# omid-arhami/topolow

Hardware: AMD Instinct MI355X
Metric: relaxation iterations/sec (NxN pairs) (higher is better)
Workload: dtype f32

## Files before the change

### include/topolow_relax.h

```cpp
#ifndef TOPOLOW_RELAX_H
#define TOPOLOW_RELAX_H

#include <stddef.h>
#include <stdint.h>

#ifdef __cplusplus
extern "C" {
#endif

#define TOPOLOW_OK 0
#define TOPOLOW_ERR_TOO_FEW_POINTS 1
#define TOPOLOW_ERR_NONFINITE 2
#define TOPOLOW_ERR_BAD_ARGUMENT 3
#define TOPOLOW_ERR_NO_DEVICE 4
#define TOPOLOW_ERR_HIP 5
#define TOPOLOW_ERR_UNSUPPORTED 6
#define TOPOLOW_ERR_INTERRUPTED 7


#define TOPOLOW_SCHEDULE_AUTO 0
#define TOPOLOW_SCHEDULE_SLAB 1
#define TOPOLOW_SCHEDULE_GS 2

#define TOPOLOW_PRECISION_AUTO 0
// ... 380 lines not shown
int topolow_session_get_positions(topolow_session* s, double* positions, char* errbuf,
                                  size_t errlen);

int topolow_session_begin(topolow_session* s, int32_t n_iter, double k0, double cooling_rate,
                          double c_repulsion, double relative_epsilon,
                          int32_t convergence_window, int32_t convergence_check_freq,
                          uint64_t seed, int32_t slab_stages, char* errbuf, size_t errlen);
int topolow_session_enqueue(topolow_session* s, int32_t max_iters, int32_t* enqueued,
                            char* errbuf, size_t errlen);
int topolow_session_wait(topolow_session* s, char* errbuf, size_t errlen);
int topolow_session_sync(topolow_session* s, int32_t* iterations_run, int32_t* stopped,
                         double* last_mae, char* errbuf, size_t errlen);
int topolow_session_finish(topolow_session* s, double* positions_out, int32_t* converged,
                           int32_t* iterations, double* final_mae, double* final_k,
                           char* errbuf, size_t errlen);
int topolow_session_check_trace(topolow_session* s, double* out, int32_t max_checks, int32_t* n_checks);
int topolow_session_hold_out(topolow_session* s, const int32_t* pair_i, const int32_t* pair_j, int64_t n_pairs,
                             const int32_t* degrees, char* errbuf, size_t errlen);
int topolow_session_restore_held_out(topolow_session* s, const int32_t* degrees, char* errbuf, size_t errlen);
int topolow_session_score_pairs(topolow_session* s, const int32_t* pair_i, const int32_t* pair_j, const double* truth,
                                int64_t n_pairs, double* sum_abs, int64_t* count, char* errbuf, size_t errlen);
int topolow_session_set_profiling(topolow_session* s, int32_t enable);
int topolow_session_profile_fused(topolow_session* s, double* fused_ms, int64_t* fused_launches, char* errbuf,
                                  size_t errlen);
int topolow_session_profile_symmetric(topolow_session* s, double* plain_ms, int64_t* plain_iterations, double* fused_ms,
                                      int64_t* fused_iterations, char* errbuf, size_t errlen);
int topolow_session_profile(topolow_session* s, double* stage_ms, int64_t* stage_launches,
                            double* check_ms, int64_t* checks, char* errbuf, size_t errlen);
int topolow_session_set_stream(topolow_session* s, void* hip_stream, int32_t external);
void* topolow_session_stream(topolow_session* s);
int32_t topolow_session_uses_dense_mae(const topolow_session* s);
int64_t topolow_session_stage_launches(const topolow_session* s);
int64_t topolow_session_checks_in_apply(const topolow_session* s);
int64_t topolow_session_bytes_per_iteration(const topolow_session* s);

int topolow_session_set_schedule(topolow_session* s, int32_t schedule);
int64_t topolow_tilegs_pair_order(int32_t n, uint64_t seed, int32_t iter, int32_t* pairs_out);
int32_t topolow_session_position_rows(const topolow_session* s);
int32_t topolow_session_position_dim(const topolow_session* s);
int topolow_session_stage(topolow_session* s, const void* d_pos_in, void* d_pos_out,
                          int32_t iter, int32_t stage, int32_t n_stages, double k,
                          char* errbuf, size_t errlen);
int topolow_session_check_partial(topolow_session* s, const void* d_pos, double* d_out2, char* errbuf,
                                  size_t errlen);
int topolow_session_controller_step(topolow_session* s, const double* d_total2, const void* d_pos,
                                    int32_t iter1, double k_after, char* errbuf, size_t errlen);
int32_t topolow_session_can_fuse_checks(const topolow_session* s);
int topolow_session_stage_fused(topolow_session* s, const void* d_pos_in, void* d_pos_out, int32_t iter,
                                double k, double* d_out2, char* errbuf, size_t errlen);
int32_t topolow_symm_segment_rows(int32_t n, int32_t segment, int32_t n_segments, int32_t* row_first,
                                  int32_t* row_end);
int32_t topolow_session_symm_segment_eligible(const topolow_session* s, int32_t n_segments);
int32_t topolow_session_can_fuse_segment_checks(const topolow_session* s);
float* topolow_session_degree_terms(topolow_session* s);
int32_t topolow_session_has_thresholds(const topolow_session* s);
int topolow_session_symm_segment_build(topolow_session* s, int32_t segment, int32_t n_segments, const void* d_rows,
                                       int32_t row_first, int32_t n_rows, int32_t any_threshold, char* errbuf,
                                       size_t errlen);
float* topolow_session_symm_moves(topolow_session* s);
int topolow_session_symm_segment_sweep(topolow_session* s, const void* d_pos_in, int32_t iter, double k,
                                       double* d_out2, char* errbuf, size_t errlen);
int topolow_session_symm_segment_apply(topolow_session* s, const void* d_pos_in, void* d_pos_out, int32_t iter,
                                       char* errbuf, size_t errlen);
int topolow_session_first_nonfinite(topolow_session* s, int32_t* iteration);
int topolow_session_edge_error(topolow_session* s, const void* d_pos, double* sum,
                               int64_t* count, char* errbuf, size_t errlen);
// ... 64 lines not shown
```

### topolow_amd/_native.py

```python
from __future__ import annotations

import ctypes as C
import math
import os
from dataclasses import dataclass, field
from typing import Any, Dict, Optional

import numpy as np

_HERE = os.path.dirname(os.path.abspath(__file__))
LIB_PATH = os.path.join(_HERE, "csrc", "libtopolow_relax.so")

SCHEDULE_AUTO, SCHEDULE_SLAB, SCHEDULE_GS = 0, 1, 2
PRECISION_AUTO, PRECISION_F32, PRECISION_F64, PRECISION_F64_EXACT = 0, 1, 2, 3

FAR_F32 = 1.0e18

OK = 0
ERR_TOO_FEW_POINTS, ERR_NONFINITE, ERR_BAD_ARGUMENT, ERR_NO_DEVICE, ERR_HIP, ERR_UNSUPPORTED, \
    ERR_INTERRUPTED = 1, 2, 3, 4, 5, 6, 7


class NativeError(RuntimeError):

# ... 193 lines not shown
    "topolow_layout_prep_fit_hist2d": (INT, (vp, dp, I32, i64p, I64, I32, I32, dp, I32, I32, dp, I32, i64p, i64p, i64p, *ERR)),
    "topolow_layout_prep_fit_linear_bins": (INT, (vp, dp, I32, i64p, I64, I32, I32, F64, F64, I32, i64p, u64p, i64p, i64p,
                                                  *ERR)),
    "topolow_session_create": (INT, (vpp, I32, I32, I32, I32, I32, I32, *ERR)),
    "topolow_session_destroy": (None, (vp,)),
    "topolow_session_set_relabel": (INT, (vp, U64, *ERR)),
    "topolow_session_labels": (INT, (vp, ip)),
    "topolow_session_load_dense": (INT, (vp, dp, ip, ip, *ERR)),
    "topolow_session_load_coo": (INT, (vp, ip, ip, dp, ip, I64, ip, *ERR)),
    "topolow_session_encoded_ptr": (devp, (vp,)),
    "topolow_session_encoded_ld": (I32, (vp,)),
    "topolow_session_commit_encoded": (INT, (vp, ip, *ERR)),
    "topolow_session_set_edges": (INT, (vp, ip, ip, dp, ip, I64, *ERR)),
    "topolow_session_set_positions": (INT, (vp, dp, *ERR)),
    "topolow_session_get_positions": (INT, (vp, dp, *ERR)),
    "topolow_session_begin": (INT, (vp, I32, F64, F64, F64, F64, I32, I32, U64, I32, *ERR)),
    "topolow_session_enqueue": (INT, (vp, I32, ip, *ERR)),
    "topolow_session_wait": (INT, (vp, *ERR)),
    "topolow_session_sync": (INT, (vp, ip, ip, dp, *ERR)),
    "topolow_session_finish": (INT, (vp, dp, ip, ip, dp, dp, *ERR)),
    "topolow_session_check_trace": (INT, (vp, dp, I32, ip)),
    "topolow_session_hold_out": (INT, (vp, ip, ip, I64, ip, *ERR)),
    "topolow_session_restore_held_out": (INT, (vp, ip, *ERR)),
    "topolow_session_score_pairs": (INT, (vp, ip, ip, dp, I64, dp, i64p, *ERR)),
    "topolow_session_set_profiling": (INT, (vp, I32)),
    "topolow_session_profile_fused": (INT, (vp, dp, i64p, *ERR)),
    "topolow_session_profile_symmetric": (INT, (vp, dp, i64p, dp, i64p, *ERR)),
    "topolow_session_profile": (INT, (vp, dp, i64p, dp, i64p, *ERR)),
    "topolow_session_set_stream": (INT, (vp, vp, I32)),
    "topolow_session_stream": (devp, (vp,)),
    "topolow_session_uses_dense_mae": (I32, (vp,)),
    "topolow_session_stage_launches": (I64, (vp,)),
    "topolow_session_checks_in_apply": (I64, (vp,)),
    "topolow_session_bytes_per_iteration": (I64, (vp,)),
    "topolow_session_set_schedule": (INT, (vp, I32)),
    "topolow_tilegs_pair_order": (I64, (I32, U64, I32, ip)),
    "topolow_session_position_rows": (I32, (vp,)),
    "topolow_session_position_dim": (I32, (vp,)),
    "topolow_session_stage": (INT, (vp, devp, devp, I32, I32, I32, F64, *ERR)),
    "topolow_session_check_partial": (INT, (vp, devp, devp, *ERR)),
    "topolow_session_controller_step": (INT, (vp, devp, devp, I32, F64, *ERR)),
    "topolow_session_can_fuse_checks": (I32, (vp,)),
    "topolow_session_stage_fused": (INT, (vp, devp, devp, I32, F64, devp, *ERR)),
    "topolow_symm_segment_rows": (I32, (I32, I32, I32, ip, ip)),
    "topolow_session_symm_segment_eligible": (I32, (vp, I32)),
    "topolow_session_can_fuse_segment_checks": (I32, (vp,)),
    "topolow_session_degree_terms": (devp, (vp,)),
    "topolow_session_has_thresholds": (I32, (vp,)),
    "topolow_session_symm_segment_build": (INT, (vp, I32, I32, devp, I32, I32, I32, *ERR)),
    "topolow_session_symm_moves": (devp, (vp,)),
    "topolow_session_symm_segment_sweep": (INT, (vp, devp, I32, F64, devp, *ERR)),
    "topolow_session_symm_segment_apply": (INT, (vp, devp, devp, I32, *ERR)),
    "topolow_session_first_nonfinite": (INT, (vp, ip)),
    "topolow_session_edge_error": (INT, (vp, devp, dp, i64p, *ERR)),
    "topolow_shard_rows": (I32, (I32, I32, I32, ip, ip)),
    "topolow_optimize_layout_exact_sharded": (INT, (dp, I32, I32, dp, ip, ip, ip, ip, dp, ip, I64, I32, F64, F64, F64, F64,
                                                    I32, I32, I32, optionsp, dp, ip, ip, dp, dp, shard_statsp, *ERR)),
    "topolow_sessions_run_sharded": (INT, (vpp, I32, dp, I32, F64, F64, F64, F64, I32, I32, U64, I32, INTERRUPT_CB, vp, I32,
                                           dp, ip, ip, dp, dp, shard_statsp, *ERR)),
    "topolow_slab_plan": (I32, (I32, I32, U64, I32, ip, I32)),
    "topolow_slab_stages_for_k": (I32, (F64, I32)),
    "topolow_symm_stage_bounds": (I32, (I32, I32, ip)),
    "topolow_symm_stage_order": (I32, (U64, I32, I32, ip)),
    "topolow_symm_stage_rows": (I32, (I32, I32, I32, ip)),
    "topolow_symm_plan": (I32, (I32, I32, I32, I32, I32, I32, ip, I32, ip)),
    "topolow_session_symm_grid": (I32, (vp,)),
# ... 1101 lines not shown
        return out.values()

    def profile_symmetric(self):
        return self._profile(self.lib.topolow_session_profile_symmetric, 2)

    def profile_fused(self):
        return self._profile(self.lib.topolow_session_profile_fused, 1)

    def set_stream(self, hip_stream, external: bool = True):
        self.lib.topolow_session_set_stream(self._h, C.c_void_p(hip_stream or None),
                                            int(bool(external)))

    @property
    def stream(self) -> int:
        return int(self.lib.topolow_session_stream(self._h) or 0)

    @property
    def position_rows(self) -> int:
        return int(self.lib.topolow_session_position_rows(self._h))

    @property
    def uses_dense_mae(self) -> bool:
        return bool(self.lib.topolow_session_uses_dense_mae(self._h))

    @property
    def stage_launches(self) -> int:
        return int(self.lib.topolow_session_stage_launches(self._h))

    @property
    def checks_in_apply(self) -> int:
        return int(self.lib.topolow_session_checks_in_apply(self._h))

    @property
    def symm_grid(self) -> int:
        return int(self.lib.topolow_session_symm_grid(self._h))

    @property
    def bytes_per_iteration(self) -> int:
        return int(self.lib.topolow_session_bytes_per_iteration(self._h))

    def stage(self, d_pos_in: int, d_pos_out: int, it: int, stage: int, n_stages: int, k: float):
        _call(self.lib.topolow_session_stage, self._h, C.c_void_p(d_pos_in), C.c_void_p(d_pos_out), int(it), int(stage),
              int(n_stages), float(k), err=self._err)

    def check_partial(self, d_pos: int, d_out2: int):
        _call(self.lib.topolow_session_check_partial, self._h, C.c_void_p(d_pos), C.c_void_p(d_out2), err=self._err)

    def controller_step(self, d_total2: int, d_pos: int, iter1: int, k_after: float):
        _call(self.lib.topolow_session_controller_step, self._h, C.c_void_p(d_total2), C.c_void_p(d_pos), int(iter1),
              float(k_after), err=self._err)

    @property
    def can_fuse_checks(self) -> bool:
        return bool(self.lib.topolow_session_can_fuse_checks(self._h))

    def stage_fused(self, d_pos_in: int, d_pos_out: int, it: int, k: float, d_out2: int):
        _call(self.lib.topolow_session_stage_fused, self._h, C.c_void_p(d_pos_in), C.c_void_p(d_pos_out), int(it), float(k),
              C.c_void_p(d_out2), err=self._err)

    @property
    def degree_terms_ptr(self) -> int:
        return int(self.lib.topolow_session_degree_terms(self._h) or 0)

    @property
    def has_thresholds(self) -> bool:
        return bool(self.lib.topolow_session_has_thresholds(self._h))
# ... 35 lines not shown
```

### topolow_amd/csrc/relax_symm.h

```cpp
#pragma once

#include <hip/hip_runtime.h>
#include <algorithm>
#include <type_traits>
#include <vector>
#include "relax_common.h"
#include "relax_kernels.h"
#include "relax_symm_plan.h"

namespace topolow {

#ifndef TOPOLOW_SYM_MINW
#define TOPOLOW_SYM_MINW 2
#endif

typedef float symf2 __attribute__((ext_vector_type(2)));
#ifdef TOPOLOW_SYM_STAMPS
__device__ unsigned long long* g_sym_stamps = nullptr;
#endif

#define TL_SYM_DPP_ADD(v, ctrl) asm volatile("v_add_f32_dpp %0, %0, %0 " ctrl " row_mask:0xf bank_mask:0xf" : "+v"(v))
template <int NV>
__device__ __forceinline__ void sym_col_reduce(float (&first)[NV], float (&second)[NV]) {
#pragma unroll
// ... 263 lines not shown
#pragma unroll
        for (int d = 0; d < DIM; ++d) {
          dst[(2 * p) * DIM + d] = racc2[p][d].x;
          dst[(2 * p + 1) * DIM + d] = racc2[p][d].y;
        }
    }
    if constexpr (ERR) {
      double s = (double)err_unit;
#pragma unroll
      for (int m = 32; m >= 1; m >>= 1) s += __shfl_xor(s, m, 64);
      if constexpr (ANYTHR) {
#pragma unroll
        for (int m = 32; m >= 1; m >>= 1) cnt_unit2 += __shfl_xor(cnt_unit2, m, 64);
      }
      if (lane == 0) {
        part_sum[slot] = s;
        part_cnt[slot] = ANYTHR ? (unsigned long long)cnt_unit2 : (slot == 0 ? fixed_cnt : 0ull);
      }
    }
  }
#ifdef TOPOLOW_SYM_STAMPS
  if (lane == 0 && g_sym_stamps != nullptr) {
    g_sym_stamps[4 * gw] = __builtin_amdgcn_s_memtime() - stamp_c0;
    g_sym_stamps[4 * gw + 1] = stamp_r0;
    g_sym_stamps[4 * gw + 2] = __builtin_amdgcn_s_memrealtime();
    unsigned hw_id, xcc_id;
    asm volatile("s_getreg_b32 %0, hwreg(HW_REG_HW_ID)" : "=s"(hw_id));
    asm volatile("s_getreg_b32 %0, hwreg(HW_REG_XCC_ID)" : "=s"(xcc_id));
    g_sym_stamps[4 * gw + 3] = ((unsigned long long)xcc_id << 32) | hw_id;
  }
#endif
}

template <int DIM, typename real> struct SymReal;
template <int DIM> struct SymReal<DIM, float> {
  static constexpr int W = SymRec<DIM>::W;
  __device__ static float ks(double k, float g) { return (float)(2.0 * k) / (4.0f * g + (float)k); }
  __device__ static float cg(double c_rep, float g) { return (float)(0.5 * c_rep) / g; }
  __device__ static float far(int) { return kFarF32; }
};

struct SymApplyCheck {
  const double* part_sum = nullptr;
  const unsigned long long* part_cnt = nullptr;
  int n_parts = 0;
  const void* pos = nullptr;
  void* best0 = nullptr;
  void* best1 = nullptr;
  long long n_values = 0;
  int check_no = 0;
  int iter1 = 0;
  double k_after = 0.0;
  double* trace = nullptr;
  int trace_cap = 0;
  RunState* mailbox = nullptr;
};

#ifndef TL_APPLY_PARTS
#define TL_APPLY_PARTS 16
#endif
constexpr int kSymApplyParts = TL_APPLY_PARTS;

template <int DIM, typename real>
__global__ __launch_bounds__(32 * kSymApplyParts) void symm_apply_kernel(
    const real* __restrict__ rec, real* __restrict__ rec_next, real* __restrict__ pos_out, const float* __restrict__ gplus,
    const real* __restrict__ rowpart, const real* __restrict__ colpart, const int2* __restrict__ row_units, int n,
// ... 210 lines not shown
```

### topolow_amd/csrc/topolow_relax.hip

```cpp

#include "topolow_session.h"
#include "topolow_prep.h"
#include "relax_kernels.h"
#include "relax_exact.h"
#include "relax_tilegs.h"
#include "relax_symm.h"
#include "relax_symm64.h"
#include "relax_symm_wide.h"
#include "relax_cv.h"

namespace {

#define TL_DISPATCH_DIM(dim, FN, ...)                 \
  switch (dim) {                                      \
    case 1: FN<1>(__VA_ARGS__); break;                \
    case 2: FN<2>(__VA_ARGS__); break;                \
    case 3: FN<3>(__VA_ARGS__); break;                \
    case 4: FN<4>(__VA_ARGS__); break;                \
    case 5: FN<5>(__VA_ARGS__); break;                \
    case 6: FN<6>(__VA_ARGS__); break;                \
    case 7: FN<7>(__VA_ARGS__); break;                \
    case 8: FN<8>(__VA_ARGS__); break;                \
    case 9: FN<9>(__VA_ARGS__); break;                \
    case 10: FN<10>(__VA_ARGS__); break;              \
// ... 555 lines not shown
  return s->sym.holds == SymHolds::kTriangle;
}

template <int DIM>
void sym_records(topolow_session* s, const void* pin, void* rec, double k) {
  sym_real<DIM>(s, [&](auto r) {
    using real = decltype(r);
    hipLaunchKernelGGL((symm_records_kernel<DIM, real>), dim3((s->sym.npad + 255) / 256), dim3(256), 0, s->stream,
                       (const real*)pin, s->gplus.p, (real*)rec, s->n, s->sym.npad, k, s->c_rep);
  });
}

template <int DIM>
void sym_sweep(topolow_session* s, const SymPlanDev& plan, const void* rec, bool thr, bool err,
               unsigned long long block_cells, int col_row0, bool prio) {
  auto& y = s->sym;
  if (err && ((size_t)plan.n_units > s->part_sum.n || (size_t)plan.n_units > s->part_cnt.n))
    throw HipError{TOPOLOW_ERR_HIP, "symmetric sweep: the error partials are smaller than the plan's unit count"};
  sym_real<DIM>(s, [&](auto r) {
    using real = decltype(r);
    sym_sweep_instance<DIM, real>(thr, err, s->exact, [&](auto kern) {
      if constexpr (std::is_same<real, double>::value)
        hipLaunchKernelGGL(kern, dim3(y.grid), dim3(64 * kSymWaves), 0, s->stream, y.tenc.p, (const double*)rec,
                           plan.units.p, plan.runs.p, (double*)y.rowpart.p, (double*)y.colpart.p, y.npad, s->state.p,
                           col_row0, y.tdelta.p, s->part_sum.p, s->part_cnt.p, block_cells);
      else
        hipLaunchKernelGGL(kern, dim3(y.grid), dim3(64 * kSymWaves), 0, s->stream, y.tenc.p, (const float*)rec,
                           plan.units.p, plan.runs.p, (float*)y.rowpart.p, (float*)y.colpart.p, y.npad, s->state.p,
                           s->part_sum.p, s->part_cnt.p, block_cells, col_row0, prio && y.prio ? 1 : 0);
    });
  });
}

bool sym_fused_ok(const topolow_session* s) {
  if (!s->sym.delta_ready) return false;
  return !s->exact || (s->list_is_block && s->n_edges > 0 && s->sym.holds == SymHolds::kTriangle);
}

template <int DIM>
void sym_apply(topolow_session* s, const SymPlanDev& plan, const void* rec, void* rec_next, void* pout, double k_next,
               int iter, int rr_stages, int rr_stage, const PendingCheck* chk = nullptr, const void* pin = nullptr,
               int n_parts = 0) {
  auto& y = s->sym;
  SymApplyCheck ac;
  if (chk != nullptr) {
    ac.part_sum = s->part_sum.p;
    ac.part_cnt = s->part_cnt.p;
    ac.n_parts = n_parts;
    ac.pos = pin;
    ac.best0 = s->best[0].p;
    ac.best1 = s->best[1].p;
    ac.check_no = s->checks_launched;
    ac.n_values = (long long)s->n * s->dim;
    ac.iter1 = chk->iter1;
    ac.k_after = chk->k_after;
    ac.trace = s->trace_dev;
    ac.trace_cap = s->trace_cap;
    ac.mailbox = s->mailbox_dev;
  }
  sym_real<DIM>(s, [&](auto r) {
    using real = decltype(r);
    hipLaunchKernelGGL((symm_apply_kernel<DIM, real>), dim3(y.npad / kSymCols + (chk != nullptr ? 1 : 0)),
                       dim3(32 * kSymApplyParts), 0, s->stream,
                       (const real*)rec, (real*)rec_next, (real*)pout, s->gplus.p, (const real*)y.rowpart.p,
                       (const real*)y.colpart.p, plan.row_units.p, s->n, y.npad, k_next, s->c_rep, iter + 1, s->state.p,
                       rr_stages, rr_stage, ac);
  });
}

bool sym_rr_stages_ok(int S) { return S == 2 || S == 4 || S == 8; }
int sym_rr_log2(int S) { return S == 2 ? 1 : (S == 4 ? 2 : 3); }

SymPlan sym_rr_plan(int npad, int n_waves, int S, int st) {
  const int TR = npad / kSymRows;
  return relax_symm_plan_rows(npad, n_waves, [&](int R, int& j0, int& j1) { sym_rr_row(TR, S, st, R, j0, j1); });
}

bool sym_rr_available(topolow_session* s, int S) {
  auto& y = s->sym;
  if (!sym_rr_stages_ok(S) || y.holds != SymHolds::kTriangle) return false;
  const int TR = y.npad / kSymRows;
  if (TR < 2 * S) return false;
  if ((long long)TR * (TR + 1) / S < (long long)y.rr_min_tiles * y.grid * kSymWaves) return false;
  const int lg = sym_rr_log2(S);
  if (!y.rr[lg].empty()) return true;
  std::vector<SymPlanDev> plans(S);
  for (int st = 0; st < S; ++st) {
    const SymPlan hp = sym_rr_plan(y.npad, y.grid * kSymWaves, S, st);
    if (hp.units.size() * kSymRows * s->dim * s->real_size() > y.rowpart.n) return false;
    plans[st].load(hp);
  }
  y.rr[lg] = std::move(plans);
  return true;
}

template <int DIM>
void sym_iteration(topolow_session* s, const void* pin, void* pout, int iter, double k, bool err, int S = 0, int st = 0,
                   bool last = true, const PendingCheck* in_apply = nullptr) {
  auto& y = s->sym;
  const SymPlanDev& plan = S == 0 ? y.plan : y.rr[sym_rr_log2(S)][st];
  ProfScope prof(s, S > 0 ? &s->prof_stage : err ? &s->prof_sym_err : &s->prof_sym);
  if (err && s->precision == TOPOLOW_PRECISION_F64 && !sym_fused_ok(s))
    throw HipError{TOPOLOW_ERR_UNSUPPORTED, "symmetric sweep (f64): no delta tiles for a fused check"};
  if (y.rec_iter != iter) {
    for (int b = 0; b < 2; ++b)
      sym_records<DIM>(s, pin, y.rec[b].p, k);
    y.rec_cur = 0;
  }
  sym_sweep<DIM>(s, plan, y.rec[y.rec_cur].p, s->any_threshold, err, S == 0 ? s->block_cells : 0ull, 0, true);
  if (in_apply != nullptr && !(err && S == 0))
    throw HipError{TOPOLOW_ERR_BAD_ARGUMENT, "symmetric sweep: a check in the apply needs the ERR sweep of a one-stage iteration"};
  sym_apply<DIM>(s, plan, y.rec[y.rec_cur].p, y.rec[y.rec_cur ^ 1].p, pout, last ? k * (1.0 - s->cooling) : k, iter, S, st,
                 in_apply, pin, plan.n_units);
  HIP_TRY(hipGetLastError());
  y.rec_cur ^= 1;
  y.rec_iter = last ? iter + 1 : iter;
  if (err) s->fused_parts = plan.n_units;
  s->stage_launches += 1;
}

enum class SymForm { kRowOwner, kSweep, kStages };
SymForm sym_form(topolow_session* s, int n_stages) {
  if (n_stages == 1) return sym_eligible(s) && sym_available(s) ? SymForm::kSweep : SymForm::kRowOwner;
  return s->sym.two_stage && sym_rr_stages_ok(n_stages) && sym_eligible(s) && sym_available(s) &&
                 sym_rr_available(s, n_stages)
             ? SymForm::kStages
             : SymForm::kRowOwner;
}

int iteration_stages(const topolow_session* s, int iter, double k) {
  return slab_geom(s->n, s->fixed_stages > 0 ? s->fixed_stages : slab_stages_at(iter, k, s->dim)).n_stages;
}

bool check_after(const topolow_session* s, int iter) { return (iter + 1) % s->check_freq == 0 || iter == s->n_iter - 1; }

struct IterPlan {
  SlabGeom geo;
  SymForm form;
  int order[8];
};
IterPlan plan_iteration(topolow_session* s, int iter, double k) {
  IterPlan p;
  p.geo = slab_geom(s->n, iteration_stages(s, iter, k));
  p.form = sym_form(s, p.geo.n_stages);
  if (p.form == SymForm::kStages) sym_rr_order(s->seed, iter, p.geo.n_stages, p.order);
  return p;
}

int enqueue_stage(topolow_session* s, const IterPlan& p, int t, const void* pin, void* pout, int iter, double k,
                  const void* push, int n_push, bool err, const PendingCheck* in_apply = nullptr) {
  if (in_apply != nullptr && p.form != SymForm::kSweep)
    throw HipError{TOPOLOW_ERR_BAD_ARGUMENT, "a check in the apply needs a one-stage symmetric sweep"};
  if (p.form == SymForm::kRowOwner) {
    TL_DISPATCH_DIM(s->dim, launch_stage, s, pin, pout, s->state.p, slab_ranges(p.geo, s->seed, iter, t), iter + 1, k,
                    push, n_push, err);
    if (err) s->fused_parts = (s->rows() + CfgProd::ROWS - 1) / CfgProd::ROWS;
  } else if (p.form == SymForm::kSweep) {
    TL_DISPATCH_SYM(s->dim, sym_iteration, s, pin, pout, iter, k, err, 0, 0, true, in_apply);
  } else {
    const int S = p.geo.n_stages;
    TL_DISPATCH_SYM(s->dim, sym_iteration, s, pin, pout, iter, k, err, S, p.order[t], t == S - 1);
  }
  return err ? s->fused_parts : 0;
}

bool check_fusable(topolow_session* s, int n_stages) {
  if (s->precision == TOPOLOW_PRECISION_F64)
    return sym_form(s, 1) == SymForm::kSweep && sym_fused_ok(s) && n_stages == 1;
  return n_stages == 1 && (s->rows() % 2 == 0 || sym_form(s, 1) == SymForm::kSweep);
}

struct SymSegment {
  long long total, t0, t1;
  int r_first = -1, r_last = -1;
};
SymSegment sym_segment(int n, int b, int P) {
  SymSegment g;
  const int npad = (n + kSymRows - 1) & ~(kSymRows - 1), TR = npad / kSymRows;
  g.total = (long long)TR * (TR + 1);
  g.t0 = g.total * b / P;
  g.t1 = g.total * (b + 1) / P;
  (void)relax_symm_plan(npad, 1, g.t0, g.t1, &g.r_first, &g.r_last);
  return g;
}

bool sym_sharded_eligible(const std::vector<topolow_session*>& ss) {
  const char* e = getenv("TOPOLOW_SHARD_SYMMETRIC");
  if (e != nullptr && e[0] == '0') return false;
  const int P = (int)ss.size();
  if (P < 2) return false;
  const topolow_session* a = ss[0];
  const long long TR = ((a->n + kSymRows - 1) & ~(kSymRows - 1)) / kSymRows;
  if (TR * (TR + 1) < 8ll * P) return false;
  for (const topolow_session* s : ss)
// ... 101 lines not shown
  if (g.r_first >= 0 && (row_first > g.r_first * kSymRows ||
                         row_first + n_rows < std::min<long long>(s->n, (long long)(g.r_last + 1) * kSymRows)))
    throw HipError{TOPOLOW_ERR_BAD_ARGUMENT, "symm_segment_build: d_rows does not hold the rows of the segment's tiles"};
  sym_build<DIM>(s, {d_rows}, {row_first, row_first + n_rows}, any_thr, g.t0, g.t1);
  sym_install_segment<DIM>(s, SymHolds::kCallerSegment, any_thr, 1, 0, {0, s->n});
}

void launch_check(topolow_session* s, PendingCheck& pc, bool error_pass) {
  hipStream_t check_on = s->stream;
  if (pc.beside) {
    HIP_TRY(hipEventRecord(s->ev_iter_done, s->stream));
    HIP_TRY(hipStreamWaitEvent(s->check_stream, s->ev_iter_done, 0));
    check_on = s->check_stream;
  }
  {
    StreamScope on(s, check_on);
    ProfScope prof(s, &s->prof_check);
    if (error_pass) {
      TL_DISPATCH_DIM(s->dim, launch_edge_error, s, s->pos[pc.buf].p, s->state.p);
      launch_controller(s, s->pos[pc.buf].p, pc.iter1, pc.k_after);
    } else {
      launch_controller(s, s->pos[pc.buf].p, pc.iter1, pc.k_after, s->part_sum.p, s->part_cnt.p, s->fused_parts);
    }
  }
  if (pc.beside) HIP_TRY(hipEventRecord(s->ev_check_done, check_on));
  hipEvent_t e = take_event(s);
  HIP_TRY(hipEventRecord(e, check_on));
  s->pending.push_back(e);
  s->checks_launched += 1;
  poll_checks(s, 3);
  pc.active = false;
}

void check_went_in_apply(topolow_session* s, PendingCheck& pc) {
  s->checks_launched += 1;
  s->checks_in_apply += 1;
  pc.active = false;
  const volatile RunState* mb = s->mailbox;
  double asked = now_s();
  while (!mb->stopped && s->checks_launched - mb->n_checks > 3) {
    if (now_s() - asked < 1e-3) continue;
    if (hipStreamQuery(s->stream) != hipErrorNotReady) break;
    (void)hipGetLastError();
    asked = now_s();
  }
  if (mb->stopped) s->host_seen_stop = true;
}

void flush_pending_check(topolow_session* s) {
  if (s->pcheck.active) launch_check(s, s->pcheck, true);
}

int nonfinite_report(int first_nonfinite, int ran, bool stopped) {
  if (first_nonfinite == 0x7fffffff) return 0;
  const int t = ((first_nonfinite + 9) / 10) * 10;
  return t <= ran && !(stopped && t == ran) ? t : 0;
}


void edges_begin(topolow_session* s, int64_t n_edges) {
  s->n_edges = n_edges;
  s->cv.list_compacted = false;
  if (s->precision == TOPOLOW_PRECISION_F64) s->sym.invalidate();
  s->n_parts = edge_error_blocks(n_edges);
  s->dense_grid_x = (((s->n + 3) & ~3) + ErrCfg::CHUNK - 1) / ErrCfg::CHUNK;
  s->dense_grid_y = (s->rows() + kErrTileRows - 1) / kErrTileRows;
  s->dense_blocks = s->dense_grid_x * s->dense_grid_y;
  const int stage_blocks = (s->rows() + CfgProd::ROWS - 1) / CfgProd::ROWS;
  int parts = std::max({s->n_parts, s->dense_blocks, stage_blocks, s->sym.plan.n_units});
  for (const auto& plans : s->sym.rr)
    for (const auto& p : plans) parts = std::max(parts, p.n_units);
  s->part_sum.alloc(parts);
  s->part_cnt.alloc(parts);
  s->dense_mae = false;
  s->dense_parity = !(s->row_begin == 0 && s->row_end == s->n);
  s->list_is_block = false;
}

bool edge_mae_forced() {
  const char* force = getenv("TOPOLOW_EDGE_MAE");
  return force && atoi(force) != 0;
}

void block_fingerprint(topolow_session* s, unsigned long long h[2]) {
  DevBuf<unsigned long long> d_fp;
  d_fp.alloc(2);
  HIP_TRY(hipMemsetAsync(d_fp.p, 0, 16, s->stream));
  hipLaunchKernelGGL(upper_fingerprint_kernel, dim3(s->rows()), dim3(kThreads), 0, s->stream,
                     s->enc.p, s->n, s->row_begin, s->row_end, s->ld, s->dense_parity ? 1 : 0,
                     d_fp.p);
  HIP_TRY(hipGetLastError());
  HIP_TRY(hipStreamSynchronize(s->stream));
  HIP_TRY(hipMemcpy(h, d_fp.p, 16, hipMemcpyDeviceToHost));
}

void edges_decide(topolow_session* s, bool list_is_block) {
  s->list_is_block = list_is_block;
  s->dense_mae = list_is_block && s->dim <= kMaxTunedDim && s->precision == TOPOLOW_PRECISION_F32;
}

bool edges_placeholders(topolow_session* s) {
  if (!s->dense_mae) return false;
  s->ei.alloc(1); s->ej.alloc(1); s->ec.alloc(1); s->et.alloc(8);
  return true;
// ... 440 lines not shown
    s->device = dev;
    s->n = n;
    s->dim = kernel_dim(ndim);
    s->udim = ndim;
    s->row_begin = row_begin;
    s->row_end = row_end;
    s->ld = (n + kEncLdAlign - 1) & ~(kEncLdAlign - 1);
    s->precision = precision == TOPOLOW_PRECISION_F64 || exact ? TOPOLOW_PRECISION_F64 : TOPOLOW_PRECISION_F32;
    s->exact = exact;
    HIP_TRY(hipStreamCreateWithFlags(&s->own_stream, hipStreamNonBlocking));
    s->stream = s->own_stream;
    HIP_TRY(hipStreamCreateWithFlags(&s->check_stream, hipStreamNonBlocking));
    HIP_TRY(hipEventCreateWithFlags(&s->ev_iter_done, hipEventDisableTiming));
    HIP_TRY(hipEventCreateWithFlags(&s->ev_check_done, hipEventDisableTiming));
    const char* serial = getenv("TOPOLOW_SERIAL_CHECKS");
    s->serial_checks = serial != nullptr && serial[0] == '1';
    const char* fuse = getenv("TOPOLOW_FUSE_CHECKS");
    s->fuse_checks = !(fuse != nullptr && fuse[0] == '0');
    const char* in_apply = getenv("TOPOLOW_CHECK_IN_APPLY");
    s->check_in_apply = !(in_apply != nullptr && in_apply[0] == '0');
    const char* symm = getenv("TOPOLOW_SYMMETRIC");
    s->sym.allowed = !(symm != nullptr && symm[0] == '0');
    s->sym.forced = symm != nullptr && symm[0] == '1';
    const char* symm_min = getenv("TOPOLOW_SYMMETRIC_MIN_N");
    s->sym.min_n = symm_min != nullptr ? atoi(symm_min) : kSymMinPoints;
    const char* symm2 = getenv("TOPOLOW_SYMMETRIC_TWO_STAGE");
    s->sym.two_stage = !(symm2 != nullptr && symm2[0] == '0');
    const char* rr_min = getenv("TOPOLOW_SYMMETRIC_STAGE_MIN_TILES");
    if (rr_min != nullptr) s->sym.rr_min_tiles = std::max(0, atoi(rr_min));
    const char* sym_grid = getenv("TOPOLOW_SYMMETRIC_GRID");
    s->sym.grid_cap = sym_grid != nullptr ? std::max(0, atoi(sym_grid)) : 0;
    const char* sym_prio = getenv("TOPOLOW_SYM_PRIO");
    s->sym.prio = !(sym_prio != nullptr && sym_prio[0] == '0');
    s->enc.alloc((size_t)((s->rows() + kEncRowAlign - 1) / kEncRowAlign * kEncRowAlign) * s->ld);
    if (s->exact) s->denc.alloc(s->enc.n);
    const size_t pos_bytes = (size_t)s->pos_rows() * s->dim * s->real_size();
    for (auto& b : s->pos) b.alloc(pos_bytes);
    for (auto& b : s->best) b.alloc(pos_bytes);
    s->state.alloc(1);
    HIP_TRY(hipHostMalloc((void**)&s->mailbox, sizeof(RunState), hipHostMallocMapped));
    std::memset(s->mailbox, 0, sizeof(RunState));
    HIP_TRY(hipHostGetDevicePointer((void**)&s->mailbox_dev, s->mailbox, 0));
  });
  if (rc != TOPOLOW_OK) { delete s; return rc; }
  *out = s;
  return TOPOLOW_OK;
}

void topolow_session_destroy(topolow_session* s) {
  if (!s) return;
  (void)hipSetDevice(s->device);
  if (s->stream) (void)hipStreamSynchronize(s->stream);
  if (s->check_stream) (void)hipStreamSynchronize(s->check_stream);
#ifdef TOPOLOW_TUNING
  g_stamps.dump();
#endif
  delete s;
}

int topolow_session_set_relabel(topolow_session* s, uint64_t seed, char* errbuf, size_t errlen) {
  if (!s) return TOPOLOW_ERR_BAD_ARGUMENT;
  if (s->gplus.p || s->part_sum.p) {
    set_err(errbuf, errlen, "the relabelling must be chosen before targets, edges or positions are loaded");
    return TOPOLOW_ERR_BAD_ARGUMENT;
  }
  return guarded(errbuf, errlen, [&] {
// ... 206 lines not shown
  return guarded(errbuf, errlen, [&] {
    HIP_TRY(hipSetDevice(s->device));
    if (!s->gplus.p) throw HipError{TOPOLOW_ERR_BAD_ARGUMENT, "session has no targets loaded"};
    if (!s->part_sum.p) throw HipError{TOPOLOW_ERR_BAD_ARGUMENT, "session has no edge list"};
    HIP_TRY(hipStreamSynchronize(s->stream));
    HIP_TRY(hipStreamSynchronize(s->check_stream));
    for (hipEvent_t e : s->pending) s->event_pool.push_back(e);
    s->pending.clear();
    s->n_iter = n_iter;
    s->k0 = k0;
    s->cooling = cooling_rate;
    s->c_rep = c_repulsion;
    s->eps = relative_epsilon;
    s->window = convergence_window;
    s->check_freq = convergence_check_freq < 1 ? 10 : convergence_check_freq;
    {
      const int need = n_iter / s->check_freq + 2;
      if (need > s->trace_cap) {
        if (s->trace) { (void)hipHostFree(s->trace); s->trace = nullptr; s->trace_cap = 0; }
        HIP_TRY(hipHostMalloc((void**)&s->trace, sizeof(double) * 3 * (size_t)need, hipHostMallocMapped));
        HIP_TRY(hipHostGetDevicePointer((void**)&s->trace_dev, s->trace, 0));
        s->trace_cap = need;
      }
    }
    s->seed = seed;
    s->fixed_stages = slab_stages;
    s->iters_enqueued = 0;
    s->k_host = k0;
    s->host_seen_stop = false;
    s->held = -1;
    s->pcheck.active = false;
    s->checks_launched = 0;
    s->checks_in_apply = 0;
    s->sym.rec_iter = -1;
    s->began = true;
    s->in_run = true;
    RunState st;
    std::memset(&st, 0, sizeof st);
    st.ctl.init(k0, convergence_window, relative_epsilon);
    st.k_base = k0;
    st.cooling = cooling_rate;
    st.n_iter = n_iter;
    st.first_nonfinite = 0x7fffffff;
    *s->mailbox = st;
    HIP_TRY(hipMemcpyAsync(s->state.p, &st, sizeof st, hipMemcpyHostToDevice, s->stream));
    HIP_TRY(hipMemcpyAsync(s->best[0].p, s->pos[s->cur].p,
                           (size_t)s->pos_rows() * s->dim * s->real_size(), hipMemcpyDeviceToDevice,
                           s->stream));
    HIP_TRY(hipStreamSynchronize(s->stream));
  });
}

int topolow_session_enqueue(topolow_session* s, int32_t max_iters, int32_t* enqueued,
                            char* errbuf, size_t errlen) {
  if (!s || !s->began) return TOPOLOW_ERR_BAD_ARGUMENT;
  if (enqueued) *enqueued = 0;
  return guarded(errbuf, errlen, [&] {
    HIP_TRY(hipSetDevice(s->device));
    int done = 0;
    while (done < max_iters && s->iters_enqueued < s->n_iter && !s->host_seen_stop) {
      const int iter = s->iters_enqueued;
      if (s->schedule == TOPOLOW_SCHEDULE_GS) {
        TL_DISPATCH_DIM(s->dim, launch_tilegs_iteration, s, s->pos[s->cur].p, iter, s->k_host);
      } else {
        const IterPlan plan = plan_iteration(s, iter, s->k_host);
        const bool fuse_now = s->pcheck.active && check_fusable(s, plan.geo.n_stages);
        if (s->pcheck.active && !fuse_now) flush_pending_check(s);
        const bool in_apply = fuse_now && s->pcheck.in_apply && plan.form == SymForm::kSweep;
        for (int t = 0; t < plan.geo.n_stages; ++t) {
          int out = 0;
          while (out == s->cur || out == s->held) ++out;
          enqueue_stage(s, plan, t, s->pos[s->cur].p, s->pos[out].p, iter, s->k_host, nullptr, 0, fuse_now,
                        in_apply ? &s->pcheck : nullptr);
          s->cur = out;
        }
        if (in_apply) check_went_in_apply(s, s->pcheck);
        else if (fuse_now) launch_check(s, s->pcheck, false);
      }
      s->iters_enqueued = iter + 1;
      s->k_host *= (1.0 - s->cooling);
      ++done;
      if (check_after(s, iter)) {
        PendingCheck pc{true, iter + 1, s->k_host, s->cur};
        pc.beside = s->schedule == TOPOLOW_SCHEDULE_SLAB && s->stream == s->own_stream &&
                    !s->profiling && !s->serial_checks;
        if (s->check_in_apply && iter + 1 == s->n_iter) pc.beside = false;
        if (s->held >= 0) HIP_TRY(hipStreamWaitEvent(s->stream, s->ev_check_done, 0));
        const bool fuse = s->fuse_checks && s->schedule == TOPOLOW_SCHEDULE_SLAB && iter + 1 < s->n_iter &&
                          (s->dense_mae || s->precision == TOPOLOW_PRECISION_F64) &&
                          check_fusable(s, iteration_stages(s, iter + 1, s->k_host));
        if (pc.beside && fuse && s->check_in_apply && sym_form(s, 1) == SymForm::kSweep) {
          pc.in_apply = true;
          pc.beside = false;
        }
        s->held = pc.beside ? s->cur : -1;
        if (fuse) s->pcheck = pc;
        else launch_check(s, pc, true);
      }
      if (s->schedule == TOPOLOW_SCHEDULE_GS && (iter + 1) % 10 == 0)
        launch_tilegs_finite(s, s->pos[s->cur].p, iter + 1);
    }
    if (enqueued) *enqueued = done;
  });
}

int topolow_session_wait(topolow_session* s, char* errbuf, size_t errlen) {
  if (!s) return TOPOLOW_ERR_BAD_ARGUMENT;
  return guarded(errbuf, errlen, [&] {
    HIP_TRY(hipSetDevice(s->device));
    HIP_TRY(hipStreamSynchronize(s->stream));
    HIP_TRY(hipStreamSynchronize(s->check_stream));
  });
}

int topolow_session_sync(topolow_session* s, int32_t* iterations_run, int32_t* stopped,
                         double* last_mae, char* errbuf, size_t errlen) {
  if (!s) return TOPOLOW_ERR_BAD_ARGUMENT;
  return guarded(errbuf, errlen, [&] {
    HIP_TRY(hipSetDevice(s->device));
    flush_pending_check(s);
    HIP_TRY(hipStreamSynchronize(s->stream));
    HIP_TRY(hipStreamSynchronize(s->check_stream));
    poll_checks(s, 0);
    RunState st;
// ... 132 lines not shown
  (void)hipStreamSynchronize(s->stream);
  (void)hipStreamSynchronize(s->check_stream);
  s->stream = external ? (hipStream_t)hip_stream : s->own_stream;
  return TOPOLOW_OK;
}

void* topolow_session_stream(topolow_session* s) { return s ? (void*)s->stream : nullptr; }

int topolow_session_set_schedule(topolow_session* s, int32_t schedule) {
  if (!s || (schedule != TOPOLOW_SCHEDULE_SLAB && schedule != TOPOLOW_SCHEDULE_GS))
    return TOPOLOW_ERR_BAD_ARGUMENT;
  if (s->row_begin != 0 || s->row_end != s->n) return TOPOLOW_ERR_UNSUPPORTED;
  s->schedule = schedule;
  return TOPOLOW_OK;
}

int64_t topolow_tilegs_pair_order(int32_t n, uint64_t seed, int32_t iter, int32_t* pairs_out) {
  return tilegs_pair_order(n, seed, iter, pairs_out);
}

int32_t topolow_session_position_rows(const topolow_session* s) { return s ? s->pos_rows() : 0; }
int32_t topolow_session_position_dim(const topolow_session* s) { return s ? s->dim : 0; }

int32_t topolow_session_uses_dense_mae(const topolow_session* s) {
  return s && s->dense_mae ? 1 : 0;
}

int64_t topolow_session_stage_launches(const topolow_session* s) {
  return s ? s->stage_launches : 0;
}

int64_t topolow_session_checks_in_apply(const topolow_session* s) {
  return s ? s->checks_in_apply : 0;
}

int64_t topolow_session_bytes_per_iteration(const topolow_session* s) {
  if (!s) return 0;
  return 4ll * s->rows() * s->n + 8ll * s->n * s->udim + 4ll * s->n;
}

int topolow_session_stage(topolow_session* s, const void* d_pos_in, void* d_pos_out,
                          int32_t iter, int32_t stage, int32_t n_stages, double k,
                          char* errbuf, size_t errlen) {
  if (!s || !d_pos_in || !d_pos_out) return TOPOLOW_ERR_BAD_ARGUMENT;
  return guarded(errbuf, errlen, [&] {
    HIP_TRY(hipSetDevice(s->device));
    const SlabGeom g = slab_geom(s->n, n_stages);
    if (stage < 0 || stage >= g.n_stages)
      throw HipError{TOPOLOW_ERR_BAD_ARGUMENT, "stage index out of range"};
    const SlabRanges rg = slab_ranges(g, s->seed, iter, stage);
    TL_DISPATCH_DIM(s->dim, launch_stage, s, d_pos_in, d_pos_out, s->began ? s->state.p : (RunState*)nullptr, rg,
                    iter + 1, k);
    s->iters_enqueued = std::max(s->iters_enqueued, iter + 1);
  });
}

int32_t topolow_session_can_fuse_checks(const topolow_session* s) {
  return s && s->fuse_checks && s->dense_mae && s->precision == TOPOLOW_PRECISION_F32 && s->rows() % 2 == 0 ? 1 : 0;
}

int topolow_session_stage_fused(topolow_session* s, const void* d_pos_in, void* d_pos_out, int32_t iter,
                                double k, double* d_out2, char* errbuf, size_t errlen) {
  if (!s || !d_pos_in || !d_pos_out || !d_out2 || !s->began) return TOPOLOW_ERR_BAD_ARGUMENT;
  if (!topolow_session_can_fuse_checks(s)) {
    set_err(errbuf, errlen, "this session cannot fuse checks (needs the fp32 block-based MAE and an even row count)");
    return TOPOLOW_ERR_UNSUPPORTED;
// ... 562 lines not shown
```

### topolow_amd/csrc/topolow_session.h

```cpp
#pragma once

#include <hip/hip_runtime.h>

#include <chrono>
#include <cstdarg>
#include <cstdio>
#include <algorithm>
#include <cstring>
#include <cstdlib>
#include <array>
#include <atomic>
#include <deque>
#include <functional>
#include <future>
#include <limits>
#include <mutex>
#include <string>
#include <memory>
#include <thread>
#include <vector>

#include "../../include/topolow_relax.h"
#include "relax_common.h"
#include "relax_host.h"
// ... 43 lines not shown
  return device;
}

double now_s() {
  return std::chrono::duration<double>(std::chrono::steady_clock::now().time_since_epoch())
      .count();
}

template <typename T>
void grow_buf(DevBuf<T>& b, size_t count) { if (b.p == nullptr || b.n < count) b.alloc(count); }

}

struct PendingCheck {
  bool active = false; int iter1 = 0; double k_after = 0.0; int buf = -1; bool beside = false; bool in_apply = false;
};

struct topolow_session {
  int n = 0, dim = 0, udim = 0, row_begin = 0, row_end = 0, ld = 0;
  int precision = TOPOLOW_PRECISION_F32;
  bool exact = false;
  int device = 0;
  hipStream_t stream = nullptr;
  hipStream_t own_stream = nullptr;
  hipStream_t check_stream = nullptr;
  hipEvent_t ev_iter_done = nullptr, ev_check_done = nullptr;
  int held = -1;
  PendingCheck pcheck;
  bool fuse_checks = true;
  bool serial_checks = false;
  bool check_in_apply = true;
  int checks_launched = 0;
  long long checks_in_apply = 0;

  std::vector<int> perm, inv;
  DevBuf<int> d_perm, d_inv;
  DevBuf<uint32_t> enc;
  DevBuf<float> denc;
  DevBuf<float> gplus;
  DevBuf<unsigned char> rowflags;
  bool any_threshold = true;
  unsigned long long block_gen = 0;
  unsigned long long block_cells = 0;
  int schedule = TOPOLOW_SCHEDULE_SLAB;
  DevBuf<int> bperm;
  DevBuf<unsigned char> pos[3];
  DevBuf<unsigned char> best[2];
  static int best_index(const RunState& st) { return st.best_buf[st.best_entry & 1] & 1; }
  void* best_now() const { return best[mailbox != nullptr ? best_index(*mailbox) : 0].p; }
  DevBuf<int> ei, ej;
  DevBuf<unsigned char> et;
  DevBuf<int8_t> ec;
  long long n_edges = 0;
  int n_parts = 0;
  bool dense_mae = false;
  bool list_is_block = false;
  bool dense_parity = false;
  int dense_blocks = 0, dense_grid_x = 0, dense_grid_y = 0;
  DevBuf<double> part_sum;
  DevBuf<unsigned long long> part_cnt;
  DevBuf<RunState> state;
  RunState* mailbox = nullptr;
  RunState* mailbox_dev = nullptr;
  double* trace = nullptr;
  double* trace_dev = nullptr;
  int trace_cap = 0;
// ... 144 lines not shown
```

Measured before the change: 19140.

## Ride convergence check on first stage of two-stage symmetric iterations

```diff
diff --git a/include/topolow_relax.h b/include/topolow_relax.h
--- a/include/topolow_relax.h
+++ b/include/topolow_relax.h
@@ -436,6 +436,8 @@
 int32_t topolow_session_uses_dense_mae(const topolow_session* s);
 int64_t topolow_session_stage_launches(const topolow_session* s);
 int64_t topolow_session_checks_in_apply(const topolow_session* s);
+int64_t topolow_session_checks_on_stages(const topolow_session* s);
+int topolow_session_fused_check_totals(topolow_session* s, double* sum2, uint64_t* count2, char* errbuf, size_t errlen);
 int64_t topolow_session_bytes_per_iteration(const topolow_session* s);
 
 int topolow_session_set_schedule(topolow_session* s, int32_t schedule);
diff --git a/topolow_amd/_native.py b/topolow_amd/_native.py
--- a/topolow_amd/_native.py
+++ b/topolow_amd/_native.py
@@ -249,6 +249,8 @@
     "topolow_session_uses_dense_mae": (I32, (vp,)),
     "topolow_session_stage_launches": (I64, (vp,)),
     "topolow_session_checks_in_apply": (I64, (vp,)),
+    "topolow_session_checks_on_stages": (I64, (vp,)),
+    "topolow_session_fused_check_totals": (INT, (vp, dp, u64p, *ERR)),
     "topolow_session_bytes_per_iteration": (I64, (vp,)),
     "topolow_session_set_schedule": (INT, (vp, I32)),
     "topolow_tilegs_pair_order": (I64, (I32, U64, I32, ip)),
@@ -1416,6 +1418,15 @@
         return int(self.lib.topolow_session_checks_in_apply(self._h))
 
     @property
+    def checks_on_stages(self) -> int:
+        return int(self.lib.topolow_session_checks_on_stages(self._h))
+
+    def fused_check_totals(self):
+        s, c = C.c_double(0.0), C.c_uint64(0)
+        _call(self.lib.topolow_session_fused_check_totals, self._h, C.byref(s), C.byref(c), err=self._err)
+        return float(s.value), int(c.value)
+
+    @property
     def symm_grid(self) -> int:
         return int(self.lib.topolow_session_symm_grid(self._h))
 
diff --git a/topolow_amd/csrc/relax_symm.h b/topolow_amd/csrc/relax_symm.h
--- a/topolow_amd/csrc/relax_symm.h
+++ b/topolow_amd/csrc/relax_symm.h
@@ -319,6 +319,106 @@
 #endif
 }
 
+template <int DIM, bool ANYTHR>
+__global__ __launch_bounds__(64 * kSymWaves, DIM <= 8 ? 4 : 3) void symm_error_kernel(
+    const uint32_t* __restrict__ enc, const float* __restrict__ rec, const SymUnit* __restrict__ units,
+    const SymRun* __restrict__ runs, const RunState* st, double* __restrict__ part_sum,
+    unsigned long long* __restrict__ part_cnt, int slot0) {
+  constexpr int W = SymRec<DIM>::W;
+  const SymRun run = runs[blockIdx.x];
+  if (st->stopped) return;
+  __shared__ double red_sum[kSymWaves];
+  __shared__ unsigned red_cnt[kSymWaves];
+  const int wave = __builtin_amdgcn_readfirstlane(threadIdx.x >> 6);
+  const int lane = threadIdx.x & 63;
+  const int a = lane & 7, b = lane >> 3;
+  const int swap = a & 1;
+  for (int u = run.u0; u < run.u1; ++u) {
+    const SymUnit U = units[u];
+    const int R = U.tile_row;
+    float pi[8][DIM];
+#pragma unroll
+    for (int r = 0; r < 8; ++r)
+#pragma unroll
+      for (int d = 0; d < DIM; ++d) pi[r][d] = rec[(size_t)(R * kSymRows + 8 * a + r) * W + d];
+    float err_unit = 0.0f;
+    unsigned cnt_unit2 = 0;
+    for (int J = U.j0 + wave; J < U.j1; J += kSymWaves) {
+      const uint4* tile = reinterpret_cast<const uint4*>(enc + (size_t)(U.tile0 + (J - U.j0)) * kSymTileWords);
+      uint4 w[8];
+#pragma unroll
+      for (int q = 0; q < 8; ++q) w[q] = tile[q * 64 + lane];
+      float err = 0.0f;
+      unsigned cnt = 0;
+#pragma unroll
+      for (int h = 0; h < 2; ++h) {
+#pragma unroll
+        for (int q = 0; q < 2; ++q) {
+          const float* cr = rec + (size_t)(J * kSymCols + 4 * b + 2 * h + (q ^ swap)) * W;
+          float pc[DIM];
+#pragma unroll
+          for (int d = 0; d < DIM; ++d) pc[d] = cr[d];
+#pragma unroll
+          for (int p = 0; p < 4; ++p)
+#pragma unroll
+            for (int e = 0; e < 2; ++e) {
+              const uint4 v = w[4 * h + p];
+              const uint32_t word = q == 0 ? (e == 0 ? v.x : v.y) : (e == 0 ? v.z : v.w);
+              float s = 0.0f;
+#pragma unroll
+              for (int d = 0; d < DIM; ++d) {
+                const float dx = pc[d] - pi[2 * p + e][d];
+                s = __builtin_fmaf(dx, dx, s);
+              }
+              const float r = __builtin_amdgcn_sqrtf(s);
+              const float t = bits_f32(ANYTHR ? (word & ~kCodeMask) : word);
+              const float diff = t - r;
+              bool sp;
+              if constexpr (ANYTHR) {
+                const uint32_t flip = (word << 30) & 0x80000000u;
+                const int32_t some = (int32_t)(((word >> 1) | word) << 31) >> 31;
+                const uint32_t k = ((f32_bits(diff) ^ flip) & (uint32_t)some) | (0x3f800000u & ~(uint32_t)some);
+                sp = bits_f32(k) > 0.0f;
+              } else {
+                sp = __builtin_amdgcn_classf(bits_f32(word), 0x1f8);
+              }
+              err += sp ? fabsf(diff) : 0.0f;
+              if constexpr (ANYTHR) cnt += sp ? 1u : 0u;
+            }
+        }
+        __builtin_amdgcn_sched_barrier(0);
+      }
+      const bool diag = J < 2 * R + 2;
+      err_unit += diag ? err : 2.0f * err;
+      cnt_unit2 += diag ? cnt : 2u * cnt;
+    }
+    double s = (double)err_unit;
+#pragma unroll
+    for (int m = 32; m >= 1; m >>= 1) s += __shfl_xor(s, m, 64);
+    if constexpr (ANYTHR) {
+#pragma unroll
+      for (int m = 32; m >= 1; m >>= 1) cnt_unit2 += __shfl_xor(cnt_unit2, m, 64);
+    }
+    if (lane == 0) {
+      red_sum[wave] = s;
+      red_cnt[wave] = cnt_unit2;
+    }
+    __syncthreads();
+    if (threadIdx.x == 0) {
+      double total = red_sum[0];
+      unsigned long long n2 = red_cnt[0];
+#pragma unroll
+      for (int q = 1; q < kSymWaves; ++q) {
+        total += red_sum[q];
+        n2 += red_cnt[q];
+      }
+      part_sum[slot0 + u] = total;
+      part_cnt[slot0 + u] = ANYTHR ? n2 : 0ull;
+    }
+    __syncthreads();
+  }
+}
+
 template <int DIM, typename real> struct SymReal;
 template <int DIM> struct SymReal<DIM, float> {
   static constexpr int W = SymRec<DIM>::W;
diff --git a/topolow_amd/csrc/topolow_relax.hip b/topolow_amd/csrc/topolow_relax.hip
--- a/topolow_amd/csrc/topolow_relax.hip
+++ b/topolow_amd/csrc/topolow_relax.hip
@@ -611,6 +611,23 @@
   });
 }
 
+template <int DIM>
+void sym_error_only(topolow_session* s, const SymPlanDev& plan, const void* rec, bool thr, int slot0) {
+  auto& y = s->sym;
+  const size_t need = (size_t)slot0 + (size_t)plan.n_units;
+  if (slot0 < 0 || need > s->part_sum.n || need > s->part_cnt.n)
+    throw HipError{TOPOLOW_ERR_HIP, "symmetric error pass: the error partials are smaller than the two plans' unit counts"};
+  if (s->precision != TOPOLOW_PRECISION_F32)
+    throw HipError{TOPOLOW_ERR_UNSUPPORTED, "symmetric error pass: fp32 sessions only"};
+  const dim3 grid(y.grid * kSymWaves), block(64 * kSymWaves);
+  if (thr)
+    hipLaunchKernelGGL((symm_error_kernel<DIM, true>), grid, block, 0, s->stream, y.tenc.p, (const float*)rec, plan.units.p,
+                       plan.runs.p, s->state.p, s->part_sum.p, s->part_cnt.p, slot0);
+  else
+    hipLaunchKernelGGL((symm_error_kernel<DIM, false>), grid, block, 0, s->stream, y.tenc.p, (const float*)rec, plan.units.p,
+                       plan.runs.p, s->state.p, s->part_sum.p, s->part_cnt.p, slot0);
+}
+
 bool sym_fused_ok(const topolow_session* s) {
   if (!s->sym.delta_ready) return false;
   return !s->exact || (s->list_is_block && s->n_edges > 0 && s->sym.holds == SymHolds::kTriangle);
@@ -669,32 +686,48 @@
     if (hp.units.size() * kSymRows * s->dim * s->real_size() > y.rowpart.n) return false;
     plans[st].load(hp);
   }
+  const size_t parts = S == 2 ? (size_t)plans[0].n_units + (size_t)plans[1].n_units : 0;
+  if (parts > s->part_sum.n || parts > s->part_cnt.n) {
+    HIP_TRY(hipStreamSynchronize(s->stream));
+    HIP_TRY(hipStreamSynchronize(s->check_stream));
+    s->part_sum.alloc(parts);
+    s->part_cnt.alloc(parts);
+  }
   y.rr[lg] = std::move(plans);
   return true;
 }
 
 template <int DIM>
 void sym_iteration(topolow_session* s, const void* pin, void* pout, int iter, double k, bool err, int S = 0, int st = 0,
-                   bool last = true, const PendingCheck* in_apply = nullptr) {
+                   bool last = true, const PendingCheck* in_apply = nullptr, int ride_other = -1) {
   auto& y = s->sym;
   const SymPlanDev& plan = S == 0 ? y.plan : y.rr[sym_rr_log2(S)][st];
   ProfScope prof(s, S > 0 ? &s->prof_stage : err ? &s->prof_sym_err : &s->prof_sym);
   if (err && s->precision == TOPOLOW_PRECISION_F64 && !sym_fused_ok(s))
     throw HipError{TOPOLOW_ERR_UNSUPPORTED, "symmetric sweep (f64): no delta tiles for a fused check"};
+  const bool rides = ride_other >= 0;
+  if (rides && !(err && S == 2 && ride_other < 2 && ride_other != st && !last && s->precision == TOPOLOW_PRECISION_F32))
+    throw HipError{TOPOLOW_ERR_BAD_ARGUMENT, "symmetric sweep: a check rides on the first stage of an fp32 two-stage iteration only"};
   if (y.rec_iter != iter) {
     for (int b = 0; b < 2; ++b)
       sym_records<DIM>(s, pin, y.rec[b].p, k);
     y.rec_cur = 0;
   }
-  sym_sweep<DIM>(s, plan, y.rec[y.rec_cur].p, s->any_threshold, err, S == 0 ? s->block_cells : 0ull, 0, true);
-  if (in_apply != nullptr && !(err && S == 0))
-    throw HipError{TOPOLOW_ERR_BAD_ARGUMENT, "symmetric sweep: a check in the apply needs the ERR sweep of a one-stage iteration"};
+  sym_sweep<DIM>(s, plan, y.rec[y.rec_cur].p, s->any_threshold, err, S == 0 || rides ? s->block_cells : 0ull, 0, true);
+  int n_parts = plan.n_units;
+  if (rides) {
+    const SymPlanDev& other = y.rr[sym_rr_log2(S)][ride_other];
+    sym_error_only<DIM>(s, other, y.rec[y.rec_cur].p, s->any_threshold, plan.n_units);
+    n_parts += other.n_units;
+  }
+  if (in_apply != nullptr && !(err && (S == 0 || rides)))
+    throw HipError{TOPOLOW_ERR_BAD_ARGUMENT, "symmetric sweep: a check in the apply needs the ERR sweep of a one-stage iteration, or of the first stage of a two-stage iteration it rides on"};
   sym_apply<DIM>(s, plan, y.rec[y.rec_cur].p, y.rec[y.rec_cur ^ 1].p, pout, last ? k * (1.0 - s->cooling) : k, iter, S, st,
-                 in_apply, pin, plan.n_units);
+                 in_apply, pin, n_parts);
   HIP_TRY(hipGetLastError());
   y.rec_cur ^= 1;
   y.rec_iter = last ? iter + 1 : iter;
-  if (err) s->fused_parts = plan.n_units;
+  if (err) s->fused_parts = n_parts;
   s->stage_launches += 1;
 }
 
@@ -726,10 +759,18 @@
   return p;
 }
 
+bool stage_check_rides(const topolow_session* s, const IterPlan& p) {
+  return s->stage_check_ride && s->fuse_checks && s->dense_mae && s->precision == TOPOLOW_PRECISION_F32 &&
+         p.form == SymForm::kStages && p.geo.n_stages == 2;
+}
+
 int enqueue_stage(topolow_session* s, const IterPlan& p, int t, const void* pin, void* pout, int iter, double k,
                   const void* push, int n_push, bool err, const PendingCheck* in_apply = nullptr) {
-  if (in_apply != nullptr && p.form != SymForm::kSweep)
-    throw HipError{TOPOLOW_ERR_BAD_ARGUMENT, "a check in the apply needs a one-stage symmetric sweep"};
+  const bool rides = err && p.form == SymForm::kStages;
+  if (rides && !(stage_check_rides(s, p) && t == 0))
+    throw HipError{TOPOLOW_ERR_BAD_ARGUMENT, "a check rides on the first stage of a two-stage symmetric iteration only"};
+  if (in_apply != nullptr && p.form != SymForm::kSweep && !rides)
+    throw HipError{TOPOLOW_ERR_BAD_ARGUMENT, "a check in the apply needs a one-stage symmetric sweep, or a two-stage iteration it rides on"};
   if (p.form == SymForm::kRowOwner) {
     TL_DISPATCH_DIM(s->dim, launch_stage, s, pin, pout, s->state.p, slab_ranges(p.geo, s->seed, iter, t), iter + 1, k,
                     push, n_push, err);
@@ -738,7 +779,8 @@
     TL_DISPATCH_SYM(s->dim, sym_iteration, s, pin, pout, iter, k, err, 0, 0, true, in_apply);
   } else {
     const int S = p.geo.n_stages;
-    TL_DISPATCH_SYM(s->dim, sym_iteration, s, pin, pout, iter, k, err, S, p.order[t], t == S - 1);
+    TL_DISPATCH_SYM(s->dim, sym_iteration, s, pin, pout, iter, k, err, S, p.order[t], t == S - 1, in_apply,
+                    rides ? p.order[1] : -1);
   }
   return err ? s->fused_parts : 0;
 }
@@ -906,9 +948,9 @@
   pc.active = false;
 }
 
-void check_went_in_apply(topolow_session* s, PendingCheck& pc) {
+void check_went_in_apply(topolow_session* s, PendingCheck& pc, bool one_stage = true) {
   s->checks_launched += 1;
-  s->checks_in_apply += 1;
+  if (one_stage) s->checks_in_apply += 1;
   pc.active = false;
   const volatile RunState* mb = s->mailbox;
   double asked = now_s();
@@ -942,8 +984,10 @@
   s->dense_blocks = s->dense_grid_x * s->dense_grid_y;
   const int stage_blocks = (s->rows() + CfgProd::ROWS - 1) / CfgProd::ROWS;
   int parts = std::max({s->n_parts, s->dense_blocks, stage_blocks, s->sym.plan.n_units});
-  for (const auto& plans : s->sym.rr)
+  for (const auto& plans : s->sym.rr) {
     for (const auto& p : plans) parts = std::max(parts, p.n_units);
+    if (plans.size() == 2) parts = std::max(parts, plans[0].n_units + plans[1].n_units);
+  }
   s->part_sum.alloc(parts);
   s->part_cnt.alloc(parts);
   s->dense_mae = false;
@@ -1450,6 +1494,8 @@
     s->sym.grid_cap = sym_grid != nullptr ? std::max(0, atoi(sym_grid)) : 0;
     const char* sym_prio = getenv("TOPOLOW_SYM_PRIO");
     s->sym.prio = !(sym_prio != nullptr && sym_prio[0] == '0');
+    const char* stage_ride = getenv("TOPOLOW_STAGE_CHECK_RIDE");
+    s->stage_check_ride = !(stage_ride != nullptr && stage_ride[0] == '0');
     s->enc.alloc((size_t)((s->rows() + kEncRowAlign - 1) / kEncRowAlign * kEncRowAlign) * s->ld);
     if (s->exact) s->denc.alloc(s->enc.n);
     const size_t pos_bytes = (size_t)s->pos_rows() * s->dim * s->real_size();
@@ -1722,6 +1768,7 @@
     s->pcheck.active = false;
     s->checks_launched = 0;
     s->checks_in_apply = 0;
+    s->checks_on_stages = 0;
     s->sym.rec_iter = -1;
     s->began = true;
     s->in_run = true;
@@ -1754,17 +1801,20 @@
         TL_DISPATCH_DIM(s->dim, launch_tilegs_iteration, s, s->pos[s->cur].p, iter, s->k_host);
       } else {
         const IterPlan plan = plan_iteration(s, iter, s->k_host);
-        const bool fuse_now = s->pcheck.active && check_fusable(s, plan.geo.n_stages);
+        const bool ride_now = s->pcheck.active && stage_check_rides(s, plan);
+        const bool fuse_now = s->pcheck.active && (ride_now || check_fusable(s, plan.geo.n_stages));
         if (s->pcheck.active && !fuse_now) flush_pending_check(s);
-        const bool in_apply = fuse_now && s->pcheck.in_apply && plan.form == SymForm::kSweep;
+        const bool in_apply = fuse_now && s->pcheck.in_apply && (ride_now || plan.form == SymForm::kSweep);
         for (int t = 0; t < plan.geo.n_stages; ++t) {
           int out = 0;
           while (out == s->cur || out == s->held) ++out;
-          enqueue_stage(s, plan, t, s->pos[s->cur].p, s->pos[out].p, iter, s->k_host, nullptr, 0, fuse_now,
-                        in_apply ? &s->pcheck : nullptr);
+          const bool carries = fuse_now && (!ride_now || t == 0);
+          enqueue_stage(s, plan, t, s->pos[s->cur].p, s->pos[out].p, iter, s->k_host, nullptr, 0, carries,
+                        in_apply && carries ? &s->pcheck : nullptr);
           s->cur = out;
         }
-        if (in_apply) check_went_in_apply(s, s->pcheck);
+        if (ride_now) s->checks_on_stages += 1;
+        if (in_apply) check_went_in_apply(s, s->pcheck, !ride_now);
         else if (fuse_now) launch_check(s, s->pcheck, false);
       }
       s->iters_enqueued = iter + 1;
@@ -1776,10 +1826,13 @@
                     !s->profiling && !s->serial_checks;
         if (s->check_in_apply && iter + 1 == s->n_iter) pc.beside = false;
         if (s->held >= 0) HIP_TRY(hipStreamWaitEvent(s->stream, s->ev_check_done, 0));
+        const bool rides = s->schedule == TOPOLOW_SCHEDULE_SLAB && iter + 1 < s->n_iter && s->stage_check_ride &&
+                           iteration_stages(s, iter + 1, s->k_host) == 2 &&
+                           stage_check_rides(s, plan_iteration(s, iter + 1, s->k_host));
         const bool fuse = s->fuse_checks && s->schedule == TOPOLOW_SCHEDULE_SLAB && iter + 1 < s->n_iter &&
                           (s->dense_mae || s->precision == TOPOLOW_PRECISION_F64) &&
-                          check_fusable(s, iteration_stages(s, iter + 1, s->k_host));
-        if (pc.beside && fuse && s->check_in_apply && sym_form(s, 1) == SymForm::kSweep) {
+                          (rides || check_fusable(s, iteration_stages(s, iter + 1, s->k_host)));
+        if (pc.beside && fuse && s->check_in_apply && (rides || sym_form(s, 1) == SymForm::kSweep)) {
           pc.in_apply = true;
           pc.beside = false;
         }
@@ -1978,6 +2031,33 @@
 
 int64_t topolow_session_checks_in_apply(const topolow_session* s) {
   return s ? s->checks_in_apply : 0;
+}
+
+int64_t topolow_session_checks_on_stages(const topolow_session* s) {
+  return s ? s->checks_on_stages : 0;
+}
+
+int topolow_session_fused_check_totals(topolow_session* s, double* sum2, uint64_t* count2, char* errbuf, size_t errlen) {
+  if (!s || !sum2 || !count2 || !s->began) return TOPOLOW_ERR_BAD_ARGUMENT;
+  return guarded(errbuf, errlen, [&] {
+    HIP_TRY(hipSetDevice(s->device));
+    HIP_TRY(hipStreamSynchronize(s->stream));
+    HIP_TRY(hipStreamSynchronize(s->check_stream));
+    const size_t parts = (size_t)std::max(s->fused_parts, 0);
+    if (parts > s->part_sum.n || parts > s->part_cnt.n)
+      throw HipError{TOPOLOW_ERR_HIP, "fused_check_totals: more partials than the buffers hold"};
+    std::vector<double> ps(parts);
+    std::vector<unsigned long long> pc(parts);
+    if (parts > 0) {
+      HIP_TRY(hipMemcpy(ps.data(), s->part_sum.p, parts * sizeof(double), hipMemcpyDeviceToHost));
+      HIP_TRY(hipMemcpy(pc.data(), s->part_cnt.p, parts * sizeof(unsigned long long), hipMemcpyDeviceToHost));
+    }
+    double sum = 0.0;
+    unsigned long long cnt = 0;
+    for (size_t q = 0; q < parts; ++q) { sum += ps[q]; cnt += pc[q]; }
+    *sum2 = sum;
+    *count2 = cnt;
+  });
 }
 
 int64_t topolow_session_bytes_per_iteration(const topolow_session* s) {
diff --git a/topolow_amd/csrc/topolow_session.h b/topolow_amd/csrc/topolow_session.h
--- a/topolow_amd/csrc/topolow_session.h
+++ b/topolow_amd/csrc/topolow_session.h
@@ -99,6 +99,8 @@
   bool check_in_apply = true;
   int checks_launched = 0;
   long long checks_in_apply = 0;
+  bool stage_check_ride = true;
+  long long checks_on_stages = 0;
 
   std::vector<int> perm, inv;
   DevBuf<int> d_perm, d_inv;
```

New measurement: 19300, median of 6. No clear change (+0.8%).
